# adeyemiadeoye/SelfConcordantSmoothOptimization.jl

Measured on AMD Instinct MI355X. Metric: iterate!() iterations/sec + achieved HBM GB/s, ProxGGNSCORE n=1M m=16k, higher is better.
Workload: dtype f64

## Files before the change

### include/scsopt.h

```cpp
#ifndef SCSOPT_H
#define SCSOPT_H

#include <stddef.h>
#include <stdint.h>

#ifdef __cplusplus
extern "C" {
#endif

#define SCS_OK 0
#define SCS_ERR_ARG 1
#define SCS_ERR_HIP 2
#define SCS_ERR_SOLVE 3
#define SCS_ERR_STATE 4
#define SCS_ERR_REF 5
#define SCS_ERR_COMM 6
#define SCS_ERR_CALLBACK 7

enum scs_loss_kind {
  SCS_LOSS_LOGISTIC_MARGIN = 1,
  SCS_LOSS_LOGISTIC_CE = 2,
  SCS_LOSS_LEAST_SQUARES = 3,
  SCS_LOSS_QUADRATIC = 4,
  SCS_LOSS_ROSENBROCK = 5,
// ... 197 lines not shown
int scs_chol_eval(scs_ctx* ctx, int64_t n, const double* M, const double* b, double* x, double* U,
                  int* info);
int scs_qr_eval(scs_ctx* ctx, int64_t n, const double* A, const double* b, double* x, double* R);
int scs_get_columns(scs_ctx* ctx, const int64_t* cols, int64_t ncols, double* out);
int scs_gram_atv_eval(scs_ctx* ctx, const double* w, const double* v, const int64_t* ij, int64_t n,
                      double* gvals, double* atv, int* fused);

int scs_multi_products_eval(scs_ctx* ctx, int K, const double* X, const double* V, double* AX, double* ATV);
int scs_multi_system_eval(scs_ctx* ctx, const double* x, double* G, int64_t ldg, double* g, double* f);
int scs_multi_sample_system_eval(scs_ctx* ctx, const double* x, double* M, int64_t ldm, double* b);

int scs_timing_enable(scs_ctx* ctx, int on);
int scs_timing_get(scs_ctx* ctx, scs_timing* out);
int scs_timing_reset(scs_ctx* ctx);
int scs_kernel_names(scs_ctx* ctx, char* gram, int64_t gram_cap, char* product, int64_t product_cap);
#define SCS_FB_LU_COOP_REFUSED 0
#define SCS_FB_LU_COOP_REDO 1
#define SCS_FB_SOLVE_BLOCKS 2
#define SCS_FB_QR_BLOCKS 3
#define SCS_FB_CHAIN_REDO 4
#define SCS_FB_PIPE_REDO 5
#define SCS_FB_QR_COOP_REFUSED 6
#define SCS_FB_QR_COOP_REDO 7
#define SCS_FB_N 8
int scs_fallback_counts(scs_ctx* ctx, int64_t* counts, int n);
int scs_sync(scs_ctx* ctx);

#ifdef __cplusplus
}
#endif
// ... 2 lines not shown
```

### selfconcordantsmoothoptimization.jl_amd/csrc/gram.hip

```cpp
#include <algorithm>
#include <cstdio>
#include <cstdlib>
#include <type_traits>
#include <vector>

#include "common.h"

namespace scs {

}
#include "gram_strip.h"
#include "gram_tiles.h"
namespace scs {

#define LDS_BARRIER()                                          \
  do {                                                         \
    asm volatile("s_waitcnt lgkmcnt(0)" ::: "memory");         \
    __builtin_amdgcn_s_barrier();                              \
    asm volatile("" ::: "memory");                             \
  } while (0)

__device__ __forceinline__ int bnd_claim(unsigned* ctr, int ntiles) {
  const int q8 = ntiles / 8, r8 = ntiles % 8;
  const int x0 = (int)((unsigned)__builtin_amdgcn_s_getreg((15 << 11) | 20) & 7u);
// ... 451 lines not shown
  int t = 0;
  for (int sbi = 0; sbi < nsb; ++sbi)
    for (int sbj = 0; sbj <= sbi; ++sbj)
      for (int i = sbi * S; i < (sbi + 1) * S && i < nb; ++i)
        for (int j = sbj * S; j < (sbj + 1) * S && j < nb; ++j)
          if (i >= j) out[t++] = make_int2(i, j);
  *ntiles = t;
}

void gram_tile_list_tall(int nb, int2* out, int* ntiles) {
  *ntiles = gram_tile_list_tall_t(nb, false, out, [](int x, int y) { return make_int2(x, y); });
}
void gram_tile_list_tall_paired(int nb, int2* out, int* ntiles) {
  *ntiles = gram_tile_list_tall_t(nb, true, out, [](int x, int y) { return make_int2(x, y); });
}

void gram_tile_list_rowmajor(int nb, int2* out) {
  int t = 0;
  for (int i = 0; i < nb; ++i)
    for (int j = 0; j <= i; ++j) out[t++] = make_int2(i, j);
}

hipError_t gram_launch_gen(const double* A1, int64_t lda1, const double* A2, int64_t lda2, const double* w,
                           int64_t k0, int64_t k1, const int2* tiles, int ntiles, double* G, int64_t ldg, int flags,
                           hipStream_t st);

template <int PIPE, int TI = 2, bool CM = false, bool AV = false, bool BND = false>
__global__ __launch_bounds__(128 * TI, (TI == 2 ? 2 : 1)) void gram_sia_kernel(
    const double* __restrict__ A, int64_t S, const double* __restrict__ w, int64_t k0, int64_t Nk,
    const int2* __restrict__ tiles, int ntiles, double* __restrict__ G, int64_t ldg, int flags,
// ... 29 lines not shown
int gram_edge_bits() {
  static const int v = env_int("SCS_GRAM_SIA", 1);
  return v >= 8 && v <= 15 ? (v & 7) : GRAM_EDGE_DEFAULT;
}
int gram_tall_mode() {
  static const int v = env_int("SCS_GRAM_GLDS", 3);
  return v;
}
int gram_addr_mode() {
  static const int v = env_int("SCS_GRAM_ADDR", 1);
  return v;
}
int gram_pair_ok() {
  static const int v = env_int("SCS_GRAM_DIAGPAIR", 1);
  return v != 0 && gram_tall_mode() == 3;
}

int gram_fuse_ok(int tall) {
  const char* e = getenv("SCS_GRAM_FUSE");
  const int mode = e ? atoi(e) : 1;
  if (mode == 0 || (!tall && mode < 2)) return 0;
  return tall ? gram_tall_mode() == 3 : gram_sia_mode() == 1;
}

__global__ void gram_vfinal_kernel(const double* __restrict__ VP, int npiece, int64_t vps, int64_t m,
                                   double* __restrict__ out) {
  const int64_t f = (int64_t)blockIdx.x * blockDim.x + threadIdx.x;
  if (f >= m) return;
  double s = VP[f];
  for (int p = 1; p < npiece; ++p) s += VP[(int64_t)p * vps + f];
// ... 219 lines not shown
                       ntiles, G, ldg, flags, nullptr, 0, 0, nullptr);
  return hipGetLastError();
}

template <int TI>
__global__ void gram_combine_kernel(const double* __restrict__ P, const int4* __restrict__ items, int nsplit,
                                    double* __restrict__ G, int64_t ldg, int packed) {
  constexpr int GTI = 64 * TI;
  const int4 it = items[blockIdx.y];
  for (int e = blockIdx.x * blockDim.x + threadIdx.x; e < GTI * GT; e += gridDim.x * blockDim.x) {
    const int jl = e / GTI, il = e % GTI;
    double sum = 0.0;
    for (int sp = 0; sp < nsplit; ++sp) sum += P[(int64_t)(it.w + sp) * GTI * GT + e];
    double* dst = (packed & 1) ? G + ((int64_t)it.z * (GTI / GT) + il / GT) * GT * GT + jl * GT + (il % GT)
                               : G + ((int64_t)it.x * GTI + il) * ldg + (int64_t)it.y * GT + jl;
    if (TI == 4 && gram_item_is_pair(it.y)) {
      int bi, bj;
      gram_item_block(it.x, it.y, il / GT, &bi, &bj);
      dst = G + ((int64_t)bi * GT + il % GT) * ldg + (int64_t)bj * GT + jl;
    }
    if (packed & 2) *dst += sum;
    else *dst = sum;
  }
}

hipError_t gram_launch_sched(const void* Av, int a32, int64_t lda, const double* w, int64_t Nk, const int4* work,
                             int seglen, int nsplit, const int4* comb, int ncomb, double* P, double* G, int64_t ldg,
                             int packed, int tall, hipStream_t st, const double* v, double* VP, int64_t vps,
                             unsigned* scnt, int sob) {
  const double* A = (const double*)Av;
  if (scnt && !(gram_fuse_ok(tall) || (tall ? gram_tall_mode() == 3 : gram_sia_mode() == 1)))
    return hipErrorInvalidValue;
  const int flags = ((packed & 1) ? GRAM_PACKED : GRAM_UPPER) | ((packed & 2) ? GRAM_ACCUMULATE : 0);
  const int glds = gram_tall_mode();
  if (v && !gram_fuse_ok(tall)) return hipErrorInvalidValue;
  if (a32) {
    const float* Af = (const float*)Av;
// ... 80 lines not shown

hipError_t gram_launch_sched_cm(const double* X, int64_t ld, const double* w, int64_t k0, int64_t k1, const int4* work,
                                int seglen, int nsplit, const int4* comb, int ncomb, double* P, double* G, int64_t ldg,
                                int flags, hipStream_t st) {
  if (seglen <= 0 || k1 <= k0) return hipSuccess;
  hipLaunchKernelGGL((gram_sia_kernel<1, 2, true>), dim3(8 * seglen), dim3(256), 0, st, X, ld, w, k0, k1, nullptr, 0,
                     G, ldg, flags | GRAM_UPPER, work, seglen, nsplit, P, nullptr, nullptr, (int64_t)0, nullptr, 0, nullptr, (int64_t)0);
  if (ncomb > 0)
    hipLaunchKernelGGL(gram_combine_kernel<2>, dim3(16, ncomb), dim3(256), 0, st, P, comb, nsplit, G, ldg,
                       (flags & GRAM_ACCUMULATE) ? 2 : 0);
  return hipGetLastError();
}

int gram_schedule(const int2* tiles, int ntiles, int slots_per_xcd, std::vector<int4>& work, std::vector<int4>& comb,
                  int* nsplit, int* npart, int diag_first_gti) {
  const int q = ntiles / 8, r = ntiles % 8;
  int tail_max = 0;
  for (int x = 0; x < 8; ++x) {
    const int n = q + (x < r ? 1 : 0);
    const int t = n % slots_per_xcd;
    tail_max = std::max(tail_max, t);
  }
  int S = 1;
  if (tail_max > 0 && 4 * tail_max < 3 * slots_per_xcd)
    S = std::max(2, std::min(16, slots_per_xcd / tail_max));
  std::vector<std::vector<int4>> seg(8);
  comb.clear();
  int pslot = 0, t0 = 0;
  for (int x = 0; x < 8; ++x) {
    const int n = q + (x < r ? 1 : 0);
    const int tail = (S > 1) ? n % slots_per_xcd : 0;
    for (int i = 0; i < n - tail; ++i) {
      const int2 tl = tiles[t0 + i];
      seg[x].push_back(make_int4(tl.x, tl.y, -1, t0 + i));
    }
    if (diag_first_gti > 0)
      std::stable_partition(seg[x].begin(), seg[x].end(), [&](const int4& it) {
        return gram_item_designated(it.x, it.y, diag_first_gti);
      });
    for (int i = n - tail; i < n; ++i) {
      const int2 tl = tiles[t0 + i];
      comb.push_back(make_int4(tl.x, tl.y, t0 + i, pslot));
      for (int sp = 0; sp < S; ++sp) seg[x].push_back(make_int4(tl.x, tl.y, sp, pslot + sp));
      pslot += S;
    }
    t0 += n;
  }
  size_t seglen = 0;
  for (auto& v : seg) seglen = std::max(seglen, v.size());
  work.assign(8 * seglen, make_int4(-1, -1, -1, -1));
  for (int x = 0; x < 8; ++x)
    for (size_t i = 0; i < seg[x].size(); ++i) work[x * seglen + i] = seg[x][i];
  *nsplit = S;
  *npart = pslot;
  return (int)seglen;
}

hipError_t gram_unpack_launch(const double* P, const int2* tiles, int ntiles, double* G, int64_t ldg,
                              hipStream_t st) {
  if (ntiles <= 0) return hipSuccess;
  hipLaunchKernelGGL(gram_packx_kernel<true>, dim3(4, ntiles), dim3(256), 0, st, P, G, tiles, ldg);
  return hipGetLastError();
}

}
```

### selfconcordantsmoothoptimization.jl_amd/csrc/gram_sia_body.h

```cpp
  static_assert(!(AV && CM), "the fused Aᵀv runs on the panel-blocked A only");
  static_assert(!CM || sizeof(TA) == sizeof(double), "column-major operands are fp64");
  constexpr int GTI = 64 * TI;
  constexpr int NT = 128 * TI;
  constexpr int FS = NT / 8;
  constexpr int NTI = 4;
  constexpr int NA = GTI / FS;
  constexpr int NB = GT / FS;
  constexpr int NMM = 2 * NTI * 4;
  constexpr int NRD = NTI + 4;
  constexpr int TAIL = NMM / 4;
  constexpr int EP = PIPE & 15;
  constexpr bool E1 = EP >= 8 && (EP & 1), E2 = EP >= 8 && (EP & 2), E3 = EP >= 8 && (EP & 4);
  constexpr bool PAIRT = TI == 4 && !CM && !BND;
  constexpr int LBR = PAIRT ? GTI : GT;
  constexpr int NAV = PAIRT ? NA : NB;
  const int packed = flags & GRAM_PACKED, accumulate = flags & GRAM_ACCUMULATE, upper = flags & GRAM_UPPER;
  __shared__ __attribute__((aligned(16))) double lds[(GTI + LBR) * GBK];
  const int orig = blockIdx.x;
  const int xcd = orig % 8;
  int bi, bj, tix, part = -1, piece = 0;
  __shared__ int s_claim;
  if constexpr (BND) {
    tix = bnd_first(scnt, (unsigned)sob, ntiles, &s_claim);
    if (tix < 0 || tix >= ntiles) return;
    bi = tiles[tix].x;
    bj = tiles[tix].y;
  } else if (work) {
    const int4 it = work[xcd * seglen + orig / 8];
    if (it.x < 0) return;
    bi = it.x;
    bj = it.y;
    tix = it.w;
// ... 2 lines not shown
      const int64_t L = ((Nk - k0 + (int64_t)nsplit * GBK - 1) / ((int64_t)nsplit * GBK)) * GBK;
      part = it.w;
      k0 = k0 + it.z * L;
      Nk = k0 + L < Nk ? k0 + L : Nk;
      if (Nk < k0) Nk = k0;
    }
  } else {
    const int q8 = ntiles / 8, r8 = ntiles % 8;
    tix = (xcd < r8 ? xcd * (q8 + 1) : r8 * (q8 + 1) + (xcd - r8) * q8) + orig / 8;
    const int2 tl = tiles[tix];
    bi = tl.x;
    bj = tl.y;
  }
bnd_tile:
  int pa = (GTI / GT) * bi, pb = pa + 1;
  bool pair = false;
  if constexpr (PAIRT) {
    if (gram_item_is_pair(bj)) {
      pair = true;
      gram_item_panels(bi, bj, &pa, &pb);
      bj = pa;
    }
  }
  int tid_ = threadIdx.x;
  if constexpr (BND) asm volatile("" : "+v"(tid_));
  const int tid = tid_, lane = tid & 63, wid = tid >> 6;
  const int wr = wid >> 1, wc = wid & 1;
  const int sc = tid & 7, sf0 = tid >> 3;
  const int64_t st0 = k0 / GBK;
  const TA* srcA = CM ? A + ((int64_t)bi * GTI + sf0) * S + k0 + 2 * sc
                      : A + ((int64_t)pa * S + st0) * GT * GBK + sf0 * GBK + 2 * sc;
  const int64_t pd = (int64_t)(pb - pa) * S * GT * GBK;
  const TA* B2 = (CM && A2) ? (const TA*)A2 : A;
  const int64_t SB2 = (CM && A2) ? S2 : S;
// ... 2 lines not shown
  const double* srcW = w + k0 + 2 * sc;
  const double* srcV = AV ? v + k0 + 2 * sc : nullptr;
  constexpr bool SB = !CM && !(PIPE & 16);
  constexpr int STB = GT * GBK * (int)sizeof(TA);
  auto uni = [](const void* p) {
    const uint64_t x = (uint64_t)p;
    const uint32_t lo = __builtin_amdgcn_readfirstlane((uint32_t)x), hi = __builtin_amdgcn_readfirstlane((uint32_t)(x >> 32));
    return (const char*)((uint64_t)hi << 32 | lo);
  };
  const char* const ubA = SB ? uni(A + ((int64_t)pa * S + st0) * GT * GBK) : nullptr;
  const char* const ubP = SB ? uni(A + ((int64_t)pb * S + st0) * GT * GBK) : nullptr;
  const char* const ubB = SB ? uni(A + ((int64_t)bj * S + st0) * GT * GBK) : nullptr;
  const char* const ubW = SB ? uni(w + k0) : nullptr;
  const char* const ubV = SB && AV ? uni(v + k0) : nullptr;
  const int vo = (sf0 * GBK + 2 * sc) * (int)sizeof(TA), vw = 2 * sc * (int)sizeof(double);
  auto window = [](const char* p, int bytes) {
    return __builtin_amdgcn_make_buffer_rsrc(const_cast<char*>(p), 0, bytes, 0x00020000);
  };
  double* la = lds;
  double* lb = lds + GTI * GBK;
  int woff[NA];
#pragma unroll
  for (int i = 0; i < NA; ++i) {
    const int f = sf0 + FS * i;
    woff[i] = f * GBK + 2 * (sc ^ swz(f));
  }
  typedef typename pair_of<TA>::type PR;
  PR ra[NA], rb[NB];
  v2d rw, rv;
  double av[NAV];
#pragma unroll
  for (int i = 0; i < NAV; ++i) av[i] = 0.0;
  auto gload = [&](int64_t st, auto fa, auto pt) {
    constexpr bool FA = decltype(fa)::value, PT = decltype(pt)::value;
    if (PIPE == 3 && st >= 2) return;
    if (CM) {
#pragma unroll
      for (int i = 0; i < NA; ++i) ra[i] = *(const PR*)(srcA + st * GBK + (int64_t)FS * i * S);
#pragma unroll
      for (int i = 0; i < NB; ++i) rb[i] = *(const PR*)(srcB + st * GBK + (int64_t)FS * i * SB2);
    } else if constexpr (SB) {
      auto bload = [](auto d, int voff, int soff) {
        if constexpr (sizeof(PR) == 16) return __builtin_bit_cast(PR, __builtin_amdgcn_raw_buffer_load_b128(d, voff, soff, 0));
        else return __builtin_bit_cast(PR, __builtin_amdgcn_raw_buffer_load_b64(d, voff, soff, 0));
      };
      const int64_t so = st * STB;
      const auto da = window(ubA + so, STB), dp = window(ubP + so, STB);
#pragma unroll
      for (int i = 0; i < NA; ++i) {
        const int f = FS * i;
        ra[i] = bload((f >> 7) ? dp : da, vo, (f & 127) * GBK * (int)sizeof(TA));
      }
      if (!PT) {
        const auto db = window(ubB + so, STB);
#pragma unroll
        for (int i = 0; i < NB; ++i) rb[i] = bload(db, vo, FS * GBK * i * (int)sizeof(TA));
      }
      constexpr int WB = GBK * (int)sizeof(double);
      rw = __builtin_bit_cast(v2d, __builtin_amdgcn_raw_buffer_load_b128(window(ubW + st * WB, WB), vw, 0, 0));
      if (FA) rv = __builtin_bit_cast(v2d, __builtin_amdgcn_raw_buffer_load_b128(window(ubV + st * WB, WB), vw, 0, 0));
      return;
    } else {
      const int64_t so = st * GT * GBK;
#pragma unroll
      for (int i = 0; i < NA; ++i) {
        const int f = FS * i;
        ra[i] = *(const PR*)(srcA + so + (f >> 7) * pd + (f & 127) * GBK);
      }
      if (!PT) {
#pragma unroll
        for (int i = 0; i < NB; ++i) rb[i] = *(const PR*)(srcB + so + FS * GBK * i);
      }
    }
    rw = *(const v2d*)(srcW + st * GBK);
    if (FA) rv = *(const v2d*)(srcV + st * GBK);
  };
  auto swrite = [&](auto fa, auto pt) {
    constexpr bool FA = decltype(fa)::value, PT = decltype(pt)::value;
#pragma unroll
    for (int i = 0; i < NA; ++i) *(v2d*)(la + woff[i]) = widen(ra[i]);
    if constexpr (PT) {
#pragma unroll
      for (int i = 0; i < NA; ++i) *(v2d*)(lb + woff[i]) = widen(ra[i]) * rw;
      if (FA) {
#pragma unroll
        for (int i = 0; i < NAV; ++i) {
          const v2d b = widen(ra[i]);
          av[i] = __builtin_fma(b[1], rv[1], __builtin_fma(b[0], rv[0], av[i]));
        }
      }
      return;
    }
#pragma unroll
    for (int i = 0; i < NB; ++i) *(v2d*)(lb + woff[i]) = widen(rb[i]) * rw;
    if (FA) {
#pragma unroll
      for (int i = 0; i < NB; ++i) {
        const v2d b = widen(rb[i]);
        av[i] = __builtin_fma(b[1], rv[1], __builtin_fma(b[0], rv[0], av[i]));
      }
    }
  };
  const int fl = lane & 15, g = lane >> 4, s = swz(fl);
  const int brow = wc * 64 + (pair ? (wr >> 1) * GT : 0);
  struct Frag {
    v2d a[NTI], b[4];
  };
  auto fread = [&](int p, Frag& F) {
    const int pc = ((4 * p + g) ^ s) * 2;
#pragma unroll
    for (int t = 0; t < NTI; ++t) F.a[t] = *(const v2d*)(la + (wr * 64 + 16 * t + fl) * GBK + pc);
#pragma unroll
    for (int t = 0; t < 4; ++t) F.b[t] = *(const v2d*)(lb + (brow + 16 * t + fl) * GBK + pc);
  };
  v4d acc[NTI][4];
#pragma unroll
  for (int i = 0; i < NTI; ++i)
#pragma unroll
    for (int j = 0; j < 4; ++j) acc[i][j] = (v4d){0.0, 0.0, 0.0, 0.0};
  auto mm = [&](const Frag& F, int n0, int n1) {
#pragma unroll
    for (int n = n0; n < n1; ++n) {
      const int u = n / (4 * NTI), ti = (n / 4) % NTI, tj = n & 3;
      acc[ti][tj] = __builtin_amdgcn_mfma_f64_16x16x4f64(F.a[ti][u], F.b[tj][u], acc[ti][tj], 0, 0, 0);
    }
  };
  auto barrier = [&]() {
    __builtin_amdgcn_sched_barrier(0);
    __builtin_amdgcn_s_waitcnt(0xC07F);
    __builtin_amdgcn_s_barrier();
    asm volatile("" ::: "memory");
    __builtin_amdgcn_sched_barrier(0);
  };
  const int nk = (int)((Nk - k0) / GBK);
  Frag F0, F1;
  auto run = [&](auto fa, auto pt) {
    constexpr int NW = decltype(pt)::value ? 2 * NA : NA + NB;
    if (nk > 0) {
      gload(0, fa, pt);
      swrite(fa, pt);
      if (nk > 1) gload(1, fa, pt);
      barrier();
      fread(0, F0);
    }
    auto body = [&](int k, bool has1, bool has2) {
      __builtin_amdgcn_sched_barrier(0);
      fread(1, F1);
      mm(F0, 0, NMM);
      if (PIPE) {
#pragma unroll
        for (int i = 0; i < NRD; ++i) {
          if (!E1) __builtin_amdgcn_sched_group_barrier(0x008, NMM / NRD, 0);
          __builtin_amdgcn_sched_group_barrier(0x100, 1, 0);
          if (E1) __builtin_amdgcn_sched_group_barrier(0x008, NMM / NRD, 0);
        }
      }
      barrier();
      if (has1) swrite(fa, pt);
      if (has2) gload(k + 2, fa, pt);
      mm(F1, 0, NMM - TAIL);
      if (PIPE) {
        if (has1) {
          constexpr int HEAD = E2 ? NMM / NRD : 0, Q = (NMM - TAIL - HEAD) / NW;
          if (E2) {
            __builtin_amdgcn_sched_group_barrier(0x008, HEAD, 0);
            __builtin_amdgcn_sched_group_barrier(0x002, 64, 0);
          }
#pragma unroll
          for (int i = 0; i < NW; ++i) {
            if (!E3) __builtin_amdgcn_sched_group_barrier(0x008, Q, 0);
            __builtin_amdgcn_sched_group_barrier(0x200, 1, 0);
            if (has2) __builtin_amdgcn_sched_group_barrier(0x020, 1, 0);
            if (E3) __builtin_amdgcn_sched_group_barrier(0x008, Q, 0);
          }
        }
        __builtin_amdgcn_sched_group_barrier(0x008, NMM, 0);
      }
      if (has1) {
        barrier();
        fread(0, F0);
      }
      mm(F1, NMM - TAIL, NMM);
      if (PIPE && has1) {
#pragma unroll
        for (int i = 0; i < NRD; ++i) {
          __builtin_amdgcn_sched_group_barrier(0x008, TAIL / NRD > 0 ? TAIL / NRD : 1, 0);
          __builtin_amdgcn_sched_group_barrier(0x100, 1, 0);
        }
      }
    };
    int k = 0;
    for (; k + 2 < nk; ++k) body(k, true, true);
    if (k + 1 < nk) {
      body(k, true, false);
      ++k;
    }
    if (k < nk) body(k, false, false);
  };
  const bool dav = AV && (pair || (int64_t)bj * GT / GTI == bi);
  if constexpr (PAIRT) {
    if (pair) run(std::bool_constant<AV>{}, std::true_type{});
    else if (dav) run(std::bool_constant<AV>{}, std::false_type{});
    else run(std::false_type{}, std::false_type{});
  } else if constexpr (AV) {
    if (dav) run(std::true_type{}, std::false_type{});
    else run(std::false_type{}, std::false_type{});
  } else {
    run(std::false_type{}, std::false_type{});
  }

  if (dav) {
#pragma unroll
    for (int i = 0; i < NAV; ++i) {
      if (i >= NB && !pair) continue;
      double t = av[i];
      t += __shfl_xor(t, 1);
      t += __shfl_xor(t, 2);
      t += __shfl_xor(t, 4);
      const int64_t row = i < NB ? (int64_t)bj * GT + sf0 + FS * i : (int64_t)pb * GT + sf0 + FS * (i - NB);
      if (sc == 0) VP[(int64_t)piece * vps + row] = t;
    }
  }

  const int pw = (wr >> 1) ? pb : pa;
  const int64_t grow = pair ? (int64_t)(pw - (wr >> 1)) * GT : (int64_t)bi * GTI;
  const int64_t gcol = pair ? (int64_t)pw * GT : (int64_t)bj * GT;
  if constexpr (BND || CM) {
#pragma unroll
    for (int ti = 0; ti < NTI; ++ti)
      gram_tile_store_row(acc[ti], ti, wr, wc, g, fl, part, P, GTI, packed, upper, accumulate, G, ldg, tix, bi, bj);
  } else {
#pragma unroll
    for (int ti = 0; ti < NTI; ++ti)
#pragma unroll
      for (int tj = 0; tj < 4; ++tj)
#pragma unroll
        for (int r = 0; r < 4; ++r) {
          const int il = wr * 64 + 16 * ti + g + 4 * r;
          const int jl = wc * 64 + 16 * tj + fl;
          double* dst;
          if (part >= 0) {
            P[((int64_t)part * GT + jl) * GTI + il] = acc[ti][tj][r];
            continue;
          }
          if (packed) dst = G + ((int64_t)tix * (GTI / GT) + il / GT) * GT * GT + jl * GT + (il % GT);
          else if (upper) dst = G + (grow + il) * ldg + gcol + jl;
          else dst = G + (gcol + jl) * ldg + grow + il;
          if (accumulate) *dst += acc[ti][tj][r];
          else *dst = acc[ti][tj][r];
        }
  }
  if (!BND && scnt && part < 0) {
    __threadfence();
    __syncthreads();
    if (tid == 0) atomicAdd(scnt + bj / sob, 1u);
  }
  if constexpr (BND) {
    tix = bnd_next(scnt, ntiles, &s_claim);
    if (tix >= ntiles) return;
    bi = tiles[tix].x;
    bj = tiles[tix].y;
    goto bnd_tile;
  }
```

### selfconcordantsmoothoptimization.jl_amd/csrc/gram_tiles.h

```cpp
#pragma once

#if defined(__HIPCC__)
#define SCS_TILES_HD __host__ __device__
#else
#define SCS_TILES_HD
#endif

namespace scs {

SCS_TILES_HD inline bool gram_item_is_pair(int y) { return y < 0; }
SCS_TILES_HD inline int gram_pair_encode(int I2) { return -1 - I2; }
SCS_TILES_HD inline int gram_pair_second(int y) { return -1 - y; }

SCS_TILES_HD inline void gram_item_panels(int x, int y, int* pa, int* pb) {
  if (gram_item_is_pair(y)) {
    *pa = 2 * x + 1;
    *pb = 2 * gram_pair_second(y) + 1;
  } else {
    *pa = 2 * x;
    *pb = 2 * x + 1;
  }
}

SCS_TILES_HD inline void gram_item_block(int x, int y, int h, int* bi, int* bj) {
  if (gram_item_is_pair(y)) {
    *bi = *bj = 2 * (h ? gram_pair_second(y) : x) + 1;
  } else {
    *bi = 2 * x + h;
    *bj = y;
  }
}

SCS_TILES_HD inline bool gram_item_designated(int x, int y, int gti) {
  return gram_item_is_pair(y) || x == (int)((long long)y * 128 / gti);
}

template <class T2, class Make>
inline int gram_tile_list_tall_t(int nb, bool pair, T2* out, Make make) {
  const int nbi = nb / 2, SI = 4, SJ = 8;
  int t = 0;
  for (int sbi = 0; sbi < (nbi + SI - 1) / SI; ++sbi)
    for (int sbj = 0; sbj <= sbi; ++sbj)
      for (int I = sbi * SI; I < (sbi + 1) * SI && I < nbi; ++I)
        for (int j = sbj * SJ; j < (sbj + 1) * SJ && j < nb; ++j) {
          if (j > 2 * I + 1) continue;
          if (pair && j == 2 * I + 1) {
            if (I % 2 == 1) continue;
            if (I + 1 < nbi) {
              out[t++] = make(I, gram_pair_encode(I + 1));
              continue;
            }
          }
          out[t++] = make(I, j);
        }
  return t;
}

}
```

### selfconcordantsmoothoptimization.jl_amd/csrc/kernels.h

```cpp
#pragma once
#include <hip/hip_runtime.h>
#include <stdint.h>

#include <vector>
#include "../../include/scsopt.h"

namespace scs {

struct ProxArgsH {
  int reg = 0;
  int use_prox = 1;
  double lam = 0.0, lam2 = 0.0;
  const double* lb = nullptr;
  const double* ub = nullptr;
  const int* gstart = nullptr;
  const int* gend = nullptr;
  const double* gw = nullptr;
  int ngroups = 0;
  const int* gmap = nullptr;
};

void gram_tile_list(int nb, int2* out, int* ntiles);
void gram_tile_list_tall(int nb, int2* out, int* ntiles);
void gram_tile_list_tall_paired(int nb, int2* out, int* ntiles);
int gram_pair_ok();
const char* gram_main_kernel_name();
hipError_t gram_launch(const void* A, int a32, int64_t lda, const double* w, int64_t Nk, const int2* tiles, int ntiles,
                       double* G, int64_t ldg, int packed, int tall, hipStream_t st, const double* v = nullptr,
                       double* VP = nullptr, int64_t vps = 0);
int gram_fuse_ok(int tall);
hipError_t gram_vfinal_launch(const double* VP, int npiece, int64_t vps, int64_t m, double* out, hipStream_t st);
void gram_tile_list_rowmajor(int nb, int2* out);
hipError_t gram_launch_gen(const double* A1, int64_t lda1, const double* A2, int64_t lda2, const double* w,
                           int64_t k0, int64_t k1, const int2* tiles, int ntiles, double* G, int64_t ldg, int flags,
                           hipStream_t st);
hipError_t gram_launch_work_cm(const double* A1, int64_t lda1, const double* A2, int64_t lda2, const double* w,
                               int64_t K, const int4* work, int seglen, int nsplit, double* P, hipStream_t st);
hipError_t gram_launch_bounded(const double* A1, int64_t lda1, const double* A2, int64_t lda2, const double* w,
                               int64_t k0, int64_t k1, const int2* tiles, int ntiles, double* G, int64_t ldg, int flags,
                               unsigned* ctr, unsigned skip, int slots, hipStream_t st, bool zeroed = false);
// ... 357 lines not shown
```

### selfconcordantsmoothoptimization.jl_amd/csrc/scsopt.cpp

```cpp
#include <hip/hip_runtime.h>
#include <rccl/rccl.h>

#include <dlfcn.h>
#include <execinfo.h>
#include <signal.h>

#include <algorithm>
#include <chrono>
#include <cmath>
#include <cstdarg>
#include <cstddef>
#include <cstdio>
#include <cstdlib>
#include <cstring>
#include <limits>
#include <atomic>
#include <condition_variable>
#include <functional>
#include <memory>
#include <mutex>
#include <string>
#include <thread>
#include <utility>
#include <vector>
// ... 151 lines not shown
  double* hloop_dev = nullptr;
  hipEvent_t loop_ev[2] = {nullptr, nullptr};
  bool dev_loop = false;
  double *G = nullptr, *Gc = nullptr;
  int2* tiles = nullptr;
  int ntiles = 0;
  int tall = 0;
  int2* utiles = nullptr;
  int nslots = 0;
  int4* gwork = nullptr;
  int4* gcomb = nullptr;
  int gseglen = 0, gncomb = 0, gnsplit = 1;
  double* gpart = nullptr;
  int2* ptiles = nullptr;
  int nptiles = 0;
  int4* pwork = nullptr;
  int4* pcomb = nullptr;
  int pseglen = 0, pncomb = 0, pnsplit = 1;
  double* vpart = nullptr;
  struct GStrip {
    int4* work = nullptr;
    int4* comb = nullptr;
    int seglen = 0, nsplit = 1, ncomb = 0;
  };
  std::vector<GStrip> gstrip;
  GStrip gpipe;
  std::vector<unsigned> gp_target;
  unsigned* gp_cnt = nullptr;
  int* gp_flag = nullptr;
  int vpieces = 1;
// ... 420 lines not shown
      ul[2 * t] = make_int2(2 * tl[t].x, tl[t].y);
      ul[2 * t + 1] = make_int2(2 * tl[t].x + 1, tl[t].y);
    }
  } else {
    gram_tile_list(nb, tl.data(), &nt);
    ul.assign(tl.begin(), tl.begin() + nt);
  }
  c->tiles = dalloc<int2>(c, nt);
  HCK(hipMemcpyAsync(c->tiles, tl.data(), sizeof(int2) * nt, hipMemcpyHostToDevice, c->st));
  c->ntiles = nt;
  c->nslots = (int)ul.size();
  std::vector<int2> tp;
  if (c->tall && gram_pair_ok()) {
    int np = 0;
    tp.resize(tl.size());
    gram_tile_list_tall_paired(nb, tp.data(), &np);
    tp.resize(np);
    c->ptiles = dalloc<int2>(c, np);
    HCK(hipMemcpyAsync(c->ptiles, tp.data(), sizeof(int2) * np, hipMemcpyHostToDevice, c->st));
    c->nptiles = np;
  }
  {
    const char* ev = std::getenv("SCS_GRAM_SCHED");
    if (!(ev && ev[0] == '0')) {
      std::vector<int4> wk, cb;
      int npart = 0, npartp = 0;
      const char* df = std::getenv("SCS_GRAM_DIAGFIRST");
      const int dfg = (df && df[0] == '0') ? 0 : c->tall ? 256 : (df && df[0] == '1') ? 128 : 0;
      c->gseglen = gram_schedule(tl.data(), nt, 32 * (c->tall ? 1 : 2), wk, cb, &c->gnsplit, &npart, dfg);
      c->gncomb = (int)cb.size();
      c->gwork = dalloc<int4>(c, wk.size());
// ... 2355 lines not shown
  dfree_t(c, c->Gd);
  dfree_t(c, c->mVt);
  c->mVt_cap = 0;
  free_view(c, c->cbv);
  dfree_t(c, c->cbstage);
  ++c->data_gen;
  dfree_t(c, c->G);
  dfree_t(c, c->Gc);
  dfree_t(c, c->tiles);
  dfree_t(c, c->utiles);
  dfree_t(c, c->gwork);
  dfree_t(c, c->gcomb);
  dfree_t(c, c->ptiles);
  dfree_t(c, c->pwork);
  dfree_t(c, c->pcomb);
  c->nptiles = c->pseglen = c->pncomb = 0;
  c->pnsplit = 1;
  dfree_t(c, c->gpart);
  dfree_t(c, c->vpart);
  for (auto& g : c->gstrip) {
    dfree_t(c, g.work);
    dfree_t(c, g.comb);
  }
  c->gstrip.clear();
  c->vpieces = 1;
  c->gseglen = c->gncomb = 0;
  c->gnsplit = 1;
  dfree_t(c, c->W);
  dfree_t(c, c->ysol);
  dfree_t(c, c->trilist);
  dfree_t(c, c->cinfo);
// ... 2337 lines not shown
  return guarded(c, [&] {
    tresolve(c);
    t->gram_ms = c->tms[T_GRAM];
    t->gram_calls = c->tcalls[T_GRAM];
    t->gemv_ms = c->tms[T_GEMV];
    t->gemv_calls = c->tcalls[T_GEMV];
    t->solve_ms = c->tms[T_SOLVE];
    t->solve_calls = c->tcalls[T_SOLVE];
    t->step_ms = c->tms[T_STEP];
    t->step_calls = c->tcalls[T_STEP];
    t->reduce_ms = c->tms[T_REDUCE];
    t->reduce_calls = c->tcalls[T_REDUCE];
  });
}

int scs_kernel_names(scs_ctx* c, char* gram, int64_t gram_cap, char* product, int64_t product_cap) {
  if (is_group(c)) return scs_kernel_names(c->subs[0], gram, gram_cap, product, product_cap);
  return guarded(c, [&] {
    auto put = [](char* dst, int64_t cap, const std::string& v) {
      if (!dst || cap <= 0) return;
      const size_t n = std::min<size_t>(v.size(), (size_t)cap - 1);
      std::memcpy(dst, v.data(), n);
      dst[n] = 0;
    };
    put(gram, gram_cap, c->gram_kname);
    put(product, product_cap, c->prod_kname);
  });
}

int scs_timing_reset(scs_ctx* c) {
// ... 459 lines not shown
```

### selfconcordantsmoothoptimization.jl_amd/scsopt/_lib.py

```python
from __future__ import annotations

import ctypes as C
import os
import sys

import numpy as np

_HERE = os.path.dirname(os.path.abspath(__file__))
LIB_PATH = os.environ.get("SCSOPT_LIB", os.path.join(_HERE, "libscsopt.so"))

SCS_OK, SCS_ERR_ARG, SCS_ERR_HIP, SCS_ERR_SOLVE, SCS_ERR_STATE, SCS_ERR_REF, SCS_ERR_COMM, SCS_ERR_CALLBACK = range(8)
SCS_MULTI_HOST_EXCHANGE = 1
SCS_CB_F, SCS_CB_GRAD, SCS_CB_HESS, SCS_CB_GGN, SCS_CB_FTEST, SCS_CB_GRAD_X = range(6)
SCS_CB_NO_METHOD = 2

SCS_SW_VALUE, SCS_SW_D1, SCS_SW_D2, SCS_SW_GGN = 1, 2, 4, 8

LOSS = {"logistic_margin": 1, "logistic_ce": 2, "least_squares": 3, "quadratic": 4, "rosenbrock": 5, "callback": 6,
        "samplewise": 7, "softmax_ce": 8, "multi_least_squares": 9}
GGN = {None: 0, "sigmoid_ce": 1, "linear_ls": 2, "samplewise": 3, "linear_softmax_ce": 4, "linear_multi_ls": 5}
REG = {"l1": 1, "l2": 2, "indbox": 3, "gl": 4}
SMOOTH = {"phuber_l1l2": 1, "phuber_indbox": 2, "phuber_gl": 3, "exp_indbox": 4, "logexp_indbox": 5, "osba_l1l2": 6,
          "osba_gl": 7}
METHOD = {"nscore": 1, "ggnscore": 2, "lqnscore": 3}
# ... 140 lines not shown
    "scs_gemv_n_eval": (C.c_int, [C.c_void_p, c_dp, c_dp]),
    "scs_solve_eval": (C.c_int, [C.c_void_p, c_dp, c_dp, c_dp, C.c_int, c_dp, C.POINTER(C.c_int)]),
    "scs_lu_eval": (C.c_int, [C.c_void_p, C.c_int64, c_dp, c_dp, c_dp, c_i32p, C.POINTER(C.c_int)]),
    "scs_chol_eval": (C.c_int, [C.c_void_p, C.c_int64, c_dp, c_dp, c_dp, c_dp, C.POINTER(C.c_int)]),
    "scs_qr_eval": (C.c_int, [C.c_void_p, C.c_int64, c_dp, c_dp, c_dp, c_dp]),
    "scs_get_columns": (C.c_int, [C.c_void_p, c_i64p, C.c_int64, c_dp]),
    "scs_gram_atv_eval": (C.c_int, [C.c_void_p, c_dp, c_dp, c_i64p, C.c_int64, c_dp, c_dp, C.POINTER(C.c_int)]),
    "scs_multi_products_eval": (C.c_int, [C.c_void_p, C.c_int, c_dp, c_dp, c_dp, c_dp]),
    "scs_multi_system_eval": (C.c_int, [C.c_void_p, c_dp, c_dp, C.c_int64, c_dp, c_dp]),
    "scs_multi_sample_system_eval": (C.c_int, [C.c_void_p, c_dp, c_dp, C.c_int64, c_dp]),
    "scs_timing_enable": (C.c_int, [C.c_void_p, C.c_int]),
    "scs_timing_get": (C.c_int, [C.c_void_p, C.POINTER(Timing)]),
    "scs_timing_reset": (C.c_int, [C.c_void_p]),
    "scs_fallback_counts": (C.c_int, [C.c_void_p, c_i64p, C.c_int]),
    "scs_kernel_names": (C.c_int, [C.c_void_p, C.c_char_p, C.c_int64, C.c_char_p, C.c_int64]),
    "scs_sync": (C.c_int, [C.c_void_p]),
}

for _name, (_res, _args) in _SIGS.items():
    _f = getattr(lib, _name)
    _f.restype = _res
    _f.argtypes = _args

EXPORTED = tuple(_SIGS)


class ScsError(RuntimeError):

    def __init__(self, code, msg):
        super().__init__(f"[scsopt rc={code}] {msg}")
# ... 221 lines not shown

    FALLBACKS = ("lu_coop_refused", "lu_coop_redo", "solve_blocks", "qr_blocks", "chain_redo", "pipe_redo",
                 "qr_coop_refused", "qr_coop_redo")

    def fallback_counts(self):
        n = len(self.FALLBACKS)
        out = (C.c_int64 * n)()
        self.check(lib.scs_fallback_counts(self.h, out, n))
        return dict(zip(self.FALLBACKS, (int(v) for v in out)))

    def kernel_names(self):
        g, p = C.create_string_buffer(128), C.create_string_buffer(128)
        self.check(lib.scs_kernel_names(self.h, g, 128, p, 128))
        return g.value.decode(), p.value.decode()

    def comm_info(self):
        k, n, r, v = C.c_int(), C.c_int(), C.c_int(), C.c_int()
        path = C.create_string_buffer(4096)
        self.check(lib.scs_comm_info(self.h, C.byref(k), C.byref(n), C.byref(r), C.byref(v), path, 4096))
        kinds = {0: "none", 1: "rccl", 2: "callback", 3: "group_rccl", 4: "group_host"}
        return {"kind": kinds.get(k.value, str(k.value)), "nranks": n.value, "rank": r.value,
                "rccl_version": v.value, "rccl_lib": path.value.decode(errors="replace")}

    def timing(self):
        t = Timing()
        self.check(lib.scs_timing_get(self.h, C.byref(t)))
        return {k: getattr(t, k) for k, _ in Timing._fields_}
```

Before: 0.2631.

## Add quad diagonal tile scheduling for tall Gram kernel with mirrored stores

Adds a new tile-list kind for the tall, paired Gram path. Diagonal 64-wide blocks are grouped into quad-S items (the lower triangle of a 4x4 diagonal block) and quad-R items (several odd diagonal blocks packed into one workgroup). The kernel gains a third load/store mode that loads all row panels into LDS once, and it mirrors stores for symmetric sub-blocks. The aim is to avoid wasted MFMA work and panel loads on the diagonal triangle tiles, at the cost of more registers and LDS, extra scheduling complexity, and duplicate writes. It is enabled by default via SCS_GRAM_DIAGQUAD.

Result: no change. 0.2614 (-0.6%).

```diff
diff --git a/include/scsopt.h b/include/scsopt.h
--- a/include/scsopt.h
+++ b/include/scsopt.h
@@ -235,6 +235,7 @@
 int scs_timing_get(scs_ctx* ctx, scs_timing* out);
 int scs_timing_reset(scs_ctx* ctx);
 int scs_kernel_names(scs_ctx* ctx, char* gram, int64_t gram_cap, char* product, int64_t product_cap);
+int scs_gram_list_info(scs_ctx* ctx, int* kind, int* items, int* nsplit);
 #define SCS_FB_LU_COOP_REFUSED 0
 #define SCS_FB_LU_COOP_REDO 1
 #define SCS_FB_SOLVE_BLOCKS 2
diff --git a/selfconcordantsmoothoptimization.jl_amd/csrc/gram.hip b/selfconcordantsmoothoptimization.jl_amd/csrc/gram.hip
--- a/selfconcordantsmoothoptimization.jl_amd/csrc/gram.hip
+++ b/selfconcordantsmoothoptimization.jl_amd/csrc/gram.hip
@@ -489,6 +489,9 @@
 void gram_tile_list_tall_paired(int nb, int2* out, int* ntiles) {
   *ntiles = gram_tile_list_tall_t(nb, true, out, [](int x, int y) { return make_int2(x, y); });
 }
+void gram_tile_list_tall_quad(int nb, int2* out, int* ntiles) {
+  *ntiles = gram_tile_list_quad_t(nb, out, [](int x, int y) { return make_int2(x, y); });
+}
 
 void gram_tile_list_rowmajor(int nb, int2* out) {
   int t = 0;
@@ -548,6 +551,10 @@
 int gram_pair_ok() {
   static const int v = env_int("SCS_GRAM_DIAGPAIR", 1);
   return v != 0 && gram_tall_mode() == 3;
+}
+int gram_quad_ok() {
+  static const int v = env_int("SCS_GRAM_DIAGQUAD", 1);
+  return v != 0 && gram_pair_ok() && gram_addr_mode() != 0;
 }
 
 int gram_fuse_ok(int tall) {
@@ -797,13 +804,24 @@
     for (int sp = 0; sp < nsplit; ++sp) sum += P[(int64_t)(it.w + sp) * GTI * GT + e];
     double* dst = (packed & 1) ? G + ((int64_t)it.z * (GTI / GT) + il / GT) * GT * GT + jl * GT + (il % GT)
                                : G + ((int64_t)it.x * GTI + il) * ldg + (int64_t)it.y * GT + jl;
+    double* dm = nullptr;
     if (TI == 4 && gram_item_is_pair(it.y)) {
       int bi, bj;
       gram_item_block(it.x, it.y, il / GT, &bi, &bj);
       dst = G + ((int64_t)bi * GT + il % GT) * ldg + (int64_t)bj * GT + jl;
+    } else if (TI == 4 && it.y < 0) {
+      int rs, cs;
+      if (!gram_quad_wave(it.x, it.y, 2 * (il / 64) + jl / 64, &rs, &cs)) continue;
+      const int64_t gr = (int64_t)rs * 64 + il % 64, gc = (int64_t)cs * 64 + jl % 64;
+      dst = G + gr * ldg + gc;
+      if (gram_quad_mirrored(rs, cs)) dm = G + gc * ldg + gr;
     }
     if (packed & 2) *dst += sum;
     else *dst = sum;
+    if (dm) {
+      if (packed & 2) *dm += sum;
+      else *dm = sum;
+    }
   }
 }
 
@@ -914,46 +932,8 @@
 
 int gram_schedule(const int2* tiles, int ntiles, int slots_per_xcd, std::vector<int4>& work, std::vector<int4>& comb,
                   int* nsplit, int* npart, int diag_first_gti) {
-  const int q = ntiles / 8, r = ntiles % 8;
-  int tail_max = 0;
-  for (int x = 0; x < 8; ++x) {
-    const int n = q + (x < r ? 1 : 0);
-    const int t = n % slots_per_xcd;
-    tail_max = std::max(tail_max, t);
-  }
-  int S = 1;
-  if (tail_max > 0 && 4 * tail_max < 3 * slots_per_xcd)
-    S = std::max(2, std::min(16, slots_per_xcd / tail_max));
-  std::vector<std::vector<int4>> seg(8);
-  comb.clear();
-  int pslot = 0, t0 = 0;
-  for (int x = 0; x < 8; ++x) {
-    const int n = q + (x < r ? 1 : 0);
-    const int tail = (S > 1) ? n % slots_per_xcd : 0;
-    for (int i = 0; i < n - tail; ++i) {
-      const int2 tl = tiles[t0 + i];
-      seg[x].push_back(make_int4(tl.x, tl.y, -1, t0 + i));
-    }
-    if (diag_first_gti > 0)
-      std::stable_partition(seg[x].begin(), seg[x].end(), [&](const int4& it) {
-        return gram_item_designated(it.x, it.y, diag_first_gti);
-      });
-    for (int i = n - tail; i < n; ++i) {
-      const int2 tl = tiles[t0 + i];
-      comb.push_back(make_int4(tl.x, tl.y, t0 + i, pslot));
-      for (int sp = 0; sp < S; ++sp) seg[x].push_back(make_int4(tl.x, tl.y, sp, pslot + sp));
-      pslot += S;
-    }
-    t0 += n;
-  }
-  size_t seglen = 0;
-  for (auto& v : seg) seglen = std::max(seglen, v.size());
-  work.assign(8 * seglen, make_int4(-1, -1, -1, -1));
-  for (int x = 0; x < 8; ++x)
-    for (size_t i = 0; i < seg[x].size(); ++i) work[x * seglen + i] = seg[x][i];
-  *nsplit = S;
-  *npart = pslot;
-  return (int)seglen;
+  return gram_schedule_t(tiles, ntiles, slots_per_xcd, work, comb, nsplit, npart, diag_first_gti,
+                         [](int x, int y, int z, int w) { return make_int4(x, y, z, w); });
 }
 
 hipError_t gram_unpack_launch(const double* P, const int2* tiles, int ntiles, double* G, int64_t ldg,
diff --git a/selfconcordantsmoothoptimization.jl_amd/csrc/gram_sia_body.h b/selfconcordantsmoothoptimization.jl_amd/csrc/gram_sia_body.h
--- a/selfconcordantsmoothoptimization.jl_amd/csrc/gram_sia_body.h
+++ b/selfconcordantsmoothoptimization.jl_amd/csrc/gram_sia_body.h
@@ -14,8 +14,12 @@
   constexpr bool PAIRT = TI == 4 && !CM && !BND;
   constexpr int LBR = PAIRT ? GTI : GT;
   constexpr int NAV = PAIRT ? NA : NB;
+  constexpr bool QUADT = PAIRT && !(PIPE & 16) && PIPE != 3;
+  constexpr int NR = 2 * GRAM_R_BLOCKS;
+  constexpr int NBX = QUADT && NR - NA > NB ? NR - NA : NB;
+  constexpr int LROWS = QUADT ? 2 * NR * 64 : GTI + LBR;
   const int packed = flags & GRAM_PACKED, accumulate = flags & GRAM_ACCUMULATE, upper = flags & GRAM_UPPER;
-  __shared__ __attribute__((aligned(16))) double lds[(GTI + LBR) * GBK];
+  __shared__ __attribute__((aligned(16))) double lds[LROWS * GBK];
   const int orig = blockIdx.x;
   const int xcd = orig % 8;
   int bi, bj, tix, part = -1, piece = 0;
@@ -48,10 +52,17 @@
   }
 bnd_tile:
   int pa = (GTI / GT) * bi, pb = pa + 1;
-  bool pair = false;
+  bool pair = false, qr = false;
+  int qy = 0;
   if constexpr (PAIRT) {
-    if (gram_item_is_pair(bj)) {
-      pair = true;
+    const int kind = gram_item_kind(bj);
+    if (kind != GRAM_TILE) {
+      if (kind != GRAM_PAIR) {
+        if constexpr (!QUADT) return;
+        qy = bj;
+      }
+      pair = kind != GRAM_QR;
+      qr = kind == GRAM_QR;
       gram_item_panels(bi, bj, &pa, &pb);
       bj = pa;
     }
@@ -84,6 +95,8 @@
   const char* const ubW = SB ? uni(w + k0) : nullptr;
   const char* const ubV = SB && AV ? uni(v + k0) : nullptr;
   const int vo = (sf0 * GBK + 2 * sc) * (int)sizeof(TA), vw = 2 * sc * (int)sizeof(double);
+  const int64_t pst = S * STB;
+  const int qn = QUADT && qr ? gram_r_count(qy) : 0;
   auto window = [](const char* p, int bytes) {
     return __builtin_amdgcn_make_buffer_rsrc(const_cast<char*>(p), 0, bytes, 0x00020000);
   };
@@ -96,13 +109,14 @@
     woff[i] = f * GBK + 2 * (sc ^ swz(f));
   }
   typedef typename pair_of<TA>::type PR;
-  PR ra[NA], rb[NB];
+  PR ra[NA], rb[NBX];
   v2d rw, rv;
   double av[NAV];
 #pragma unroll
   for (int i = 0; i < NAV; ++i) av[i] = 0.0;
   auto gload = [&](int64_t st, auto fa, auto pt) {
-    constexpr bool FA = decltype(fa)::value, PT = decltype(pt)::value;
+    constexpr bool FA = decltype(fa)::value;
+    constexpr int PT = decltype(pt)::value;
     if (PIPE == 3 && st >= 2) return;
     if (CM) {
 #pragma unroll
@@ -115,11 +129,19 @@
         else return __builtin_bit_cast(PR, __builtin_amdgcn_raw_buffer_load_b64(d, voff, soff, 0));
       };
       const int64_t so = st * STB;
+      if constexpr (PT == 2) {
+#pragma unroll
+        for (int i = 0; i < NR; ++i) {
+          const auto d = window(ubA + so + i * pst, i / 2 < qn ? STB : 0);
+          (i < NA ? ra[i] : rb[i - NA]) = bload(d, vo, 64 * GBK * (int)sizeof(TA));
+        }
+      } else {
       const auto da = window(ubA + so, STB), dp = window(ubP + so, STB);
 #pragma unroll
       for (int i = 0; i < NA; ++i) {
         const int f = FS * i;
         ra[i] = bload((f >> 7) ? dp : da, vo, (f & 127) * GBK * (int)sizeof(TA));
+      }
       }
       if (!PT) {
         const auto db = window(ubB + so, STB);
@@ -146,10 +168,22 @@
     if (FA) rv = *(const v2d*)(srcV + st * GBK);
   };
   auto swrite = [&](auto fa, auto pt) {
-    constexpr bool FA = decltype(fa)::value, PT = decltype(pt)::value;
+    constexpr bool FA = decltype(fa)::value;
+    constexpr int PT = decltype(pt)::value;
+    if constexpr (PT == 2) {
+      int lbo = woff[0] + NR * 64 * GBK;
+      asm volatile("" : "+v"(lbo));
+#pragma unroll
+      for (int i = 0; i < NR; ++i) {
+        const v2d c = widen(i < NA ? ra[i] : rb[i - NA]);
+        *(v2d*)(la + woff[i % NA] + (i / NA) * GTI * GBK) = c;
+        *(v2d*)(la + lbo + i * FS * GBK) = c * rw;
+      }
+      return;
+    }
 #pragma unroll
     for (int i = 0; i < NA; ++i) *(v2d*)(la + woff[i]) = widen(ra[i]);
-    if constexpr (PT) {
+    if constexpr (PT == 1) {
 #pragma unroll
       for (int i = 0; i < NA; ++i) *(v2d*)(lb + woff[i]) = widen(ra[i]) * rw;
       if (FA) {
@@ -172,16 +206,26 @@
     }
   };
   const int fl = lane & 15, g = lane >> 4, s = swz(fl);
-  const int brow = wc * 64 + (pair ? (wr >> 1) * GT : 0);
+  int aslab = wr, bslab = wc + (pair ? (wr >> 1) * (GT / 64) : 0);
+  int qrs = 0, qcs = 0;
+  bool qlive = true;
+  if constexpr (QUADT) {
+    if (qy) {
+      qlive = gram_quad_wave(bi, qy, wid, &qrs, &qcs);
+      aslab = qr ? wid : qrs - 4 * bi;
+      bslab = qr ? wid : qcs - 4 * bi;
+    }
+  }
   struct Frag {
     v2d a[NTI], b[4];
   };
-  auto fread = [&](int p, Frag& F) {
+  auto fread = [&](int p, Frag& F, auto pt) {
+    const double* const lbp = decltype(pt)::value == 2 ? lds + NR * 64 * GBK : lb;
     const int pc = ((4 * p + g) ^ s) * 2;
 #pragma unroll
-    for (int t = 0; t < NTI; ++t) F.a[t] = *(const v2d*)(la + (wr * 64 + 16 * t + fl) * GBK + pc);
-#pragma unroll
-    for (int t = 0; t < 4; ++t) F.b[t] = *(const v2d*)(lb + (brow + 16 * t + fl) * GBK + pc);
+    for (int t = 0; t < NTI; ++t) F.a[t] = *(const v2d*)(la + (aslab * 64 + 16 * t + fl) * GBK + pc);
+#pragma unroll
+    for (int t = 0; t < 4; ++t) F.b[t] = *(const v2d*)(lbp + (bslab * 64 + 16 * t + fl) * GBK + pc);
   };
   v4d acc[NTI][4];
 #pragma unroll
@@ -205,17 +249,18 @@
   const int nk = (int)((Nk - k0) / GBK);
   Frag F0, F1;
   auto run = [&](auto fa, auto pt) {
-    constexpr int NW = decltype(pt)::value ? 2 * NA : NA + NB;
+    constexpr int PT = decltype(pt)::value;
+    constexpr int NW = PT == 2 ? 2 * NR : PT ? 2 * NA : NA + NB;
     if (nk > 0) {
       gload(0, fa, pt);
       swrite(fa, pt);
       if (nk > 1) gload(1, fa, pt);
       barrier();
-      fread(0, F0);
+      fread(0, F0, pt);
     }
     auto body = [&](int k, bool has1, bool has2) {
       __builtin_amdgcn_sched_barrier(0);
-      fread(1, F1);
+      fread(1, F1, pt);
       mm(F0, 0, NMM);
       if (PIPE) {
 #pragma unroll
@@ -234,13 +279,15 @@
           constexpr int HEAD = E2 ? NMM / NRD : 0, Q = (NMM - TAIL - HEAD) / NW;
           if (E2) {
             __builtin_amdgcn_sched_group_barrier(0x008, HEAD, 0);
-            __builtin_amdgcn_sched_group_barrier(0x002, 64, 0);
+            if (PT != 2) __builtin_amdgcn_sched_group_barrier(0x002, 64, 0);
           }
 #pragma unroll
           for (int i = 0; i < NW; ++i) {
             if (!E3) __builtin_amdgcn_sched_group_barrier(0x008, Q, 0);
+            if (PT == 2) __builtin_amdgcn_sched_group_barrier(0x002, 2, 0);
             __builtin_amdgcn_sched_group_barrier(0x200, 1, 0);
-            if (has2) __builtin_amdgcn_sched_group_barrier(0x020, 1, 0);
+            if (has2 && (PT != 2 || (i & 1))) __builtin_amdgcn_sched_group_barrier(0x020, 1, 0);
+            if (has2 && PT == 2 && i == NW - 1) __builtin_amdgcn_sched_group_barrier(0x020, 1, 0);
             if (E3) __builtin_amdgcn_sched_group_barrier(0x008, Q, 0);
           }
         }
@@ -248,7 +295,7 @@
       }
       if (has1) {
         barrier();
-        fread(0, F0);
+        fread(0, F0, pt);
       }
       mm(F1, NMM - TAIL, NMM);
       if (PIPE && has1) {
@@ -267,16 +314,27 @@
     }
     if (k < nk) body(k, false, false);
   };
-  const bool dav = AV && (pair || (int64_t)bj * GT / GTI == bi);
+  const bool dav = AV && !qr && (pair || (int64_t)bj * GT / GTI == bi);
+  using PT0 = std::integral_constant<int, 0>;
+  using PT1 = std::integral_constant<int, 1>;
+  using PT2 = std::integral_constant<int, 2>;
   if constexpr (PAIRT) {
-    if (pair) run(std::bool_constant<AV>{}, std::true_type{});
-    else if (dav) run(std::bool_constant<AV>{}, std::false_type{});
-    else run(std::false_type{}, std::false_type{});
+    bool ran = false;
+    if constexpr (QUADT) {
+      if (qr) {
+        run(std::false_type{}, PT2{});
+        ran = true;
+      }
+    }
+    if (ran) {
+    } else if (pair) run(std::bool_constant<AV>{}, PT1{});
+    else if (dav) run(std::bool_constant<AV>{}, PT0{});
+    else run(std::false_type{}, PT0{});
   } else if constexpr (AV) {
-    if (dav) run(std::true_type{}, std::false_type{});
-    else run(std::false_type{}, std::false_type{});
+    if (dav) run(std::true_type{}, PT0{});
+    else run(std::false_type{}, PT0{});
   } else {
-    run(std::false_type{}, std::false_type{});
+    run(std::false_type{}, PT0{});
   }
 
   if (dav) {
@@ -293,13 +351,21 @@
   }
 
   const int pw = (wr >> 1) ? pb : pa;
-  const int64_t grow = pair ? (int64_t)(pw - (wr >> 1)) * GT : (int64_t)bi * GTI;
-  const int64_t gcol = pair ? (int64_t)pw * GT : (int64_t)bj * GT;
+  int64_t grow = pair ? (int64_t)(pw - (wr >> 1)) * GT : (int64_t)bi * GTI;
+  int64_t gcol = pair ? (int64_t)pw * GT : (int64_t)bj * GT;
+  bool qmir = false;
+  if constexpr (QUADT) {
+    if (qy) {
+      grow = (int64_t)(qrs - wr) * 64;
+      gcol = (int64_t)(qcs - wc) * 64;
+      qmir = part < 0 && gram_quad_mirrored(qrs, qcs);
+    }
+  }
   if constexpr (BND || CM) {
 #pragma unroll
     for (int ti = 0; ti < NTI; ++ti)
       gram_tile_store_row(acc[ti], ti, wr, wc, g, fl, part, P, GTI, packed, upper, accumulate, G, ldg, tix, bi, bj);
-  } else {
+  } else if (qlive) {
 #pragma unroll
     for (int ti = 0; ti < NTI; ++ti)
 #pragma unroll
@@ -318,6 +384,13 @@
           else dst = G + (gcol + jl) * ldg + grow + il;
           if (accumulate) *dst += acc[ti][tj][r];
           else *dst = acc[ti][tj][r];
+          if constexpr (QUADT) {
+            if (qmir) {
+              double* const dm = upper ? G + (gcol + jl) * ldg + grow + il : G + (grow + il) * ldg + gcol + jl;
+              if (accumulate) *dm += acc[ti][tj][r];
+              else *dm = acc[ti][tj][r];
+            }
+          }
         }
   }
   if (!BND && scnt && part < 0) {
diff --git a/selfconcordantsmoothoptimization.jl_amd/csrc/gram_tiles.h b/selfconcordantsmoothoptimization.jl_amd/csrc/gram_tiles.h
--- a/selfconcordantsmoothoptimization.jl_amd/csrc/gram_tiles.h
+++ b/selfconcordantsmoothoptimization.jl_amd/csrc/gram_tiles.h
@@ -1,4 +1,7 @@
 #pragma once
+
+#include <algorithm>
+#include <vector>
 
 #if defined(__HIPCC__)
 #define SCS_TILES_HD __host__ __device__
@@ -8,9 +11,31 @@
 
 namespace scs {
 
-SCS_TILES_HD inline bool gram_item_is_pair(int y) { return y < 0; }
+enum { GRAM_TILE = 0, GRAM_PAIR = 1, GRAM_QS = 2, GRAM_QR = 3 };
+constexpr int GRAM_Y_SPAN = 1 << 24;
+constexpr int GRAM_Y_S = -GRAM_Y_SPAN - 1;
+constexpr int GRAM_Y_R = -GRAM_Y_SPAN - 2;
+constexpr int GRAM_R_BLOCKS = 4;
+SCS_TILES_HD inline int gram_item_kind(int y) {
+  return y >= 0 ? GRAM_TILE : y >= -GRAM_Y_SPAN ? GRAM_PAIR : y == GRAM_Y_S ? GRAM_QS : GRAM_QR;
+}
+SCS_TILES_HD inline bool gram_item_is_pair(int y) { return y < 0 && y >= -GRAM_Y_SPAN; }
 SCS_TILES_HD inline int gram_pair_encode(int I2) { return -1 - I2; }
 SCS_TILES_HD inline int gram_pair_second(int y) { return -1 - y; }
+SCS_TILES_HD inline int gram_r_encode(int n) { return GRAM_Y_R - (n - 1); }
+SCS_TILES_HD inline int gram_r_count(int y) { return GRAM_Y_R - y + 1; }
+
+SCS_TILES_HD inline bool gram_quad_wave(int x, int y, int wave, int* rs, int* cs) {
+  if (gram_item_kind(y) == GRAM_QS) {
+    const unsigned QA = 0x33322210u, QB = 0x21021000u;
+    *rs = 4 * x + (int)((QA >> (4 * wave)) & 15u);
+    *cs = 4 * x + (int)((QB >> (4 * wave)) & 15u);
+    return true;
+  }
+  *rs = *cs = 4 * (x + wave / 2) + 1 + 2 * (wave & 1);
+  return wave / 2 < gram_r_count(y);
+}
+SCS_TILES_HD inline bool gram_quad_mirrored(int rs, int cs) { return rs == cs + 1 && (cs & 1) == 0; }
 
 SCS_TILES_HD inline void gram_item_panels(int x, int y, int* pa, int* pb) {
   if (gram_item_is_pair(y)) {
@@ -32,7 +57,9 @@
 }
 
 SCS_TILES_HD inline bool gram_item_designated(int x, int y, int gti) {
-  return gram_item_is_pair(y) || x == (int)((long long)y * 128 / gti);
+  const int kind = gram_item_kind(y);
+  if (kind != GRAM_TILE) return kind != GRAM_QR;
+  return x == (int)((long long)y * 128 / gti);
 }
 
 template <class T2, class Make>
@@ -56,4 +83,66 @@
   return t;
 }
 
+template <class T2, class Make>
+inline int gram_tile_list_quad_t(int nb, T2* out, Make make) {
+  const int nbi = nb / 2, SI = 4, SJ = 8;
+  int t = 0;
+  for (int sbi = 0; sbi < (nbi + SI - 1) / SI; ++sbi)
+    for (int sbj = 0; sbj <= sbi; ++sbj)
+      for (int I = sbi * SI; I < (sbi + 1) * SI && I < nbi; ++I)
+        for (int j = sbj * SJ; j < (sbj + 1) * SJ && j < nb; ++j) {
+          if (j > 2 * I + 1) continue;
+          if (j == 2 * I) out[t++] = make(I, (int)GRAM_Y_S);
+          else if (j < 2 * I) out[t++] = make(I, j);
+          else if (I % GRAM_R_BLOCKS == 0)
+            out[t++] = make(I, gram_r_encode(nbi - I < GRAM_R_BLOCKS ? nbi - I : GRAM_R_BLOCKS));
+        }
+  return t;
 }
+
+template <class T2, class T4, class Make4>
+inline int gram_schedule_t(const T2* tiles, int ntiles, int slots_per_xcd, std::vector<T4>& work, std::vector<T4>& comb,
+                           int* nsplit, int* npart, int diag_first_gti, Make4 make4) {
+  const int q = ntiles / 8, r = ntiles % 8;
+  int tail_max = 0;
+  for (int x = 0; x < 8; ++x) {
+    const int n = q + (x < r ? 1 : 0);
+    const int t = n % slots_per_xcd;
+    tail_max = std::max(tail_max, t);
+  }
+  int S = 1;
+  if (tail_max > 0 && 4 * tail_max < 3 * slots_per_xcd)
+    S = std::max(2, std::min(16, slots_per_xcd / tail_max));
+  std::vector<std::vector<T4>> seg(8);
+  comb.clear();
+  int pslot = 0, t0 = 0;
+  for (int x = 0; x < 8; ++x) {
+    const int n = q + (x < r ? 1 : 0);
+    const int tail = (S > 1) ? n % slots_per_xcd : 0;
+    for (int i = 0; i < n - tail; ++i) {
+      const T2 tl = tiles[t0 + i];
+      seg[x].push_back(make4(tl.x, tl.y, -1, t0 + i));
+    }
+    if (diag_first_gti > 0)
+      std::stable_partition(seg[x].begin(), seg[x].end(), [&](const T4& it) {
+        return gram_item_designated(it.x, it.y, diag_first_gti);
+      });
+    for (int i = n - tail; i < n; ++i) {
+      const T2 tl = tiles[t0 + i];
+      comb.push_back(make4(tl.x, tl.y, t0 + i, pslot));
+      for (int sp = 0; sp < S; ++sp) seg[x].push_back(make4(tl.x, tl.y, sp, pslot + sp));
+      pslot += S;
+    }
+    t0 += n;
+  }
+  size_t seglen = 0;
+  for (auto& v : seg) seglen = std::max(seglen, v.size());
+  work.assign(8 * seglen, make4(-1, -1, -1, -1));
+  for (int x = 0; x < 8; ++x)
+    for (size_t i = 0; i < seg[x].size(); ++i) work[x * seglen + i] = seg[x][i];
+  *nsplit = S;
+  *npart = pslot;
+  return (int)seglen;
+}
+
+}
diff --git a/selfconcordantsmoothoptimization.jl_amd/csrc/kernels.h b/selfconcordantsmoothoptimization.jl_amd/csrc/kernels.h
--- a/selfconcordantsmoothoptimization.jl_amd/csrc/kernels.h
+++ b/selfconcordantsmoothoptimization.jl_amd/csrc/kernels.h
@@ -24,6 +24,8 @@
 void gram_tile_list_tall(int nb, int2* out, int* ntiles);
 void gram_tile_list_tall_paired(int nb, int2* out, int* ntiles);
 int gram_pair_ok();
+void gram_tile_list_tall_quad(int nb, int2* out, int* ntiles);
+int gram_quad_ok();
 const char* gram_main_kernel_name();
 hipError_t gram_launch(const void* A, int a32, int64_t lda, const double* w, int64_t Nk, const int2* tiles, int ntiles,
                        double* G, int64_t ldg, int packed, int tall, hipStream_t st, const double* v = nullptr,
diff --git a/selfconcordantsmoothoptimization.jl_amd/csrc/scsopt.cpp b/selfconcordantsmoothoptimization.jl_amd/csrc/scsopt.cpp
--- a/selfconcordantsmoothoptimization.jl_amd/csrc/scsopt.cpp
+++ b/selfconcordantsmoothoptimization.jl_amd/csrc/scsopt.cpp
@@ -189,6 +189,7 @@
   double* gpart = nullptr;
   int2* ptiles = nullptr;
   int nptiles = 0;
+  int pkind = 0;
   int4* pwork = nullptr;
   int4* pcomb = nullptr;
   int pseglen = 0, pncomb = 0, pnsplit = 1;
@@ -639,7 +640,9 @@
   if (c->tall && gram_pair_ok()) {
     int np = 0;
     tp.resize(tl.size());
-    gram_tile_list_tall_paired(nb, tp.data(), &np);
+    c->pkind = gram_quad_ok() ? 2 : 1;
+    if (c->pkind == 2) gram_tile_list_tall_quad(nb, tp.data(), &np);
+    else gram_tile_list_tall_paired(nb, tp.data(), &np);
     tp.resize(np);
     c->ptiles = dalloc<int2>(c, np);
     HCK(hipMemcpyAsync(c->ptiles, tp.data(), sizeof(int2) * np, hipMemcpyHostToDevice, c->st));
@@ -3025,7 +3028,7 @@
   dfree_t(c, c->ptiles);
   dfree_t(c, c->pwork);
   dfree_t(c, c->pcomb);
-  c->nptiles = c->pseglen = c->pncomb = 0;
+  c->nptiles = c->pseglen = c->pncomb = c->pkind = 0;
   c->pnsplit = 1;
   dfree_t(c, c->gpart);
   dfree_t(c, c->vpart);
@@ -5393,6 +5396,15 @@
   });
 }
 
+int scs_gram_list_info(scs_ctx* c, int* kind, int* items, int* nsplit) {
+  if (is_group(c)) return scs_gram_list_info(c->subs[0], kind, items, nsplit);
+  return guarded(c, [&] {
+    if (kind) *kind = c->ptiles ? c->pkind : 0;
+    if (items) *items = c->ptiles ? c->nptiles : c->ntiles;
+    if (nsplit) *nsplit = !c->gwork ? 1 : c->ptiles ? c->pnsplit : c->gnsplit;
+  });
+}
+
 int scs_kernel_names(scs_ctx* c, char* gram, int64_t gram_cap, char* product, int64_t product_cap) {
   if (is_group(c)) return scs_kernel_names(c->subs[0], gram, gram_cap, product, product_cap);
   return guarded(c, [&] {
diff --git a/selfconcordantsmoothoptimization.jl_amd/scsopt/_lib.py b/selfconcordantsmoothoptimization.jl_amd/scsopt/_lib.py
--- a/selfconcordantsmoothoptimization.jl_amd/scsopt/_lib.py
+++ b/selfconcordantsmoothoptimization.jl_amd/scsopt/_lib.py
@@ -178,6 +178,7 @@
     "scs_timing_reset": (C.c_int, [C.c_void_p]),
     "scs_fallback_counts": (C.c_int, [C.c_void_p, c_i64p, C.c_int]),
     "scs_kernel_names": (C.c_int, [C.c_void_p, C.c_char_p, C.c_int64, C.c_char_p, C.c_int64]),
+    "scs_gram_list_info": (C.c_int, [C.c_void_p, C.POINTER(C.c_int), C.POINTER(C.c_int), C.POINTER(C.c_int)]),
     "scs_sync": (C.c_int, [C.c_void_p]),
 }
 
@@ -429,6 +430,11 @@
         self.check(lib.scs_kernel_names(self.h, g, 128, p, 128))
         return g.value.decode(), p.value.decode()
 
+    def gram_list_info(self):
+        k, n, s = C.c_int(), C.c_int(), C.c_int()
+        self.check(lib.scs_gram_list_info(self.h, C.byref(k), C.byref(n), C.byref(s)))
+        return ("tiles", "paired", "quad")[k.value], n.value, s.value
+
     def comm_info(self):
         k, n, r, v = C.c_int(), C.c_int(), C.c_int(), C.c_int()
         path = C.create_string_buffer(4096)
```
